# ittiam-systems/libxaac

Hardware: AMD Instinct MI355X
Metric: decoded audio frames/s (1024-spl IMDCT + complex QMF + HQ SBR + parametric stereo, HE-AACv2) (higher is better)
Workload: dtype int32

## Files before the change

### libxaac_amd/csrc/sbr_core_kernel.hip

```cpp
#include <hip/hip_runtime.h>
#include <stddef.h>
#include <stdint.h>
#include <stdlib.h>

#ifdef XS_PROFILE
__shared__ long long xs_prof_last[4];
__shared__ unsigned xs_prof_acc[4][32];
#define XS_T(i)                                                  \
  do {                                                           \
    if ((threadIdx.x & 63) == 0) {                               \
      long long t_ = clock64();                                  \
      xs_prof_acc[threadIdx.x >> 6][i] += (unsigned)(t_ - xs_prof_last[threadIdx.x >> 6]); \
      xs_prof_last[threadIdx.x >> 6] = t_;                       \
    }                                                            \
  } while (0)
#endif
__shared__ int16_t xs_lds_inv_table[256];
__shared__ int16_t xs_lds_sqrt_table[258];
__shared__ int32_t xs_lds_rand_ph[568];
__shared__ int16_t xs_lds_rand_hi[568];
__shared__ int16_t xs_lds_small16[8 + 4 + 50];
__shared__ int32_t xs_lds_new_bw[16];
#define XS_TAB_LIMG(i) xs_lds_small16[i]
#define XS_TAB_SMOOTH(i) xs_lds_small16[8 + (i)]
#define XS_TAB_INVINT(i) xs_lds_small16[12 + (i)]
#define XS_TAB_NEWBW(i) xs_lds_new_bw[i]
#define XS_TAB_RAND(i) xs_lds_rand_ph[i]
#define XS_SYNC_WAVE_LDS 1
#define XS_TAB_INV(i) xs_lds_inv_table[i]
#define XS_TAB_SQRT(i) xs_lds_sqrt_table[i]
#include "sbr_core.h"
#include "sbr_core_kernel.h"

#ifndef XS_STAGGER_G
#define XS_STAGGER_G 64
#endif
#ifndef XS_STAGGER_SLEEP
#define XS_STAGGER_SLEEP 16
#endif

namespace {

__device__ __forceinline__ void xs_wave_sync() {
  __builtin_amdgcn_fence(__ATOMIC_RELEASE, "wavefront");
  __builtin_amdgcn_wave_barrier();
  __builtin_amdgcn_fence(__ATOMIC_ACQUIRE, "wavefront");
}

struct XsLdsState {
  int16_t codec_usb, syn_lsb, syn_usb, pad2_;
  XAAC_SBR_STATE_TAIL_FIELDS
};
constexpr int kHeadOff = offsetof(xaac_sbr_state, codec_usb);
constexpr int kTailOff = offsetof(xaac_sbr_state, lpc_real);
constexpr int kTailWords = (sizeof(xaac_sbr_state) - kTailOff) / 4;
static_assert(kHeadOff % 4 == 0 && kTailOff % 4 == 0 && sizeof(xaac_sbr_state) % 4 == 0, "word copies");
static_assert(offsetof(XsLdsState, lpc_real) == 8 && sizeof(XsLdsState) == 8 + kTailWords * 4, "mirror layout");
static_assert(offsetof(xaac_sbr_state, overlap) % 16 == 0 || true, "");
static_assert(sizeof(xaac_sbr_header) % 4 == 0 && sizeof(xaac_sbr_frame) % 4 == 0, "word copies");

constexpr int kFrameHeadBytes = offsetof(xaac_sbr_frame, int_env_sf_arr);
static_assert(kFrameHeadBytes % 4 == 0 && offsetof(xaac_sbr_frame, int_noise_floor) % 4 == 0, "word copies");
static_assert(offsetof(xaac_sbr_frame, int_noise_floor) == kFrameHeadBytes + sizeof(((xaac_sbr_frame *)0)->int_env_sf_arr),
              "nothing but the two arrays behind the head");

template <int HQ, int NB>
struct XsLds {
  typedef XsQmfT<HQ, NB> Q;
  int32_t x[XAAC_SBR_X_ROWS * Q::ROW + (HQ ? 0 : 128)];
  XsLdsState st;
  xaac_sbr_header h;
  int32_t f_head[kFrameHeadBytes / 4];
  int32_t noise_floor[sizeof(((xaac_sbr_frame *)0)->int_noise_floor) / 4];
  XsWork w;
#ifdef XS_LDS_PAD
  char occupancy_probe[XS_LDS_PAD];
#endif
};

__device__ __forceinline__ void copy_words(int32_t *dst, const int32_t *src, int n, int lane) {
  int i = lane;
  for (; i + 64 * 7 < n; i += 64 * 8) {
    int32_t t[8];
#pragma unroll
    for (int j = 0; j < 8; j++) t[j] = src[i + 64 * j];
#pragma unroll
    for (int j = 0; j < 8; j++) dst[i + 64 * j] = t[j];
  }
  int32_t t[8];
#pragma unroll
  for (int j = 0; j < 8; j++)
    if (i + 64 * j < n) t[j] = src[i + 64 * j];
#pragma unroll
  for (int j = 0; j < 8; j++)
    if (i + 64 * j < n) dst[i + 64 * j] = t[j];
}

template <int HQ, int NB, int NS = 32>
__device__ __forceinline__ bool core_one(const XaacSbrCoreParams &p, const int ch, XsLds<HQ, NB> &s, const int lane) {
  typedef XsQmfT<HQ, NB, 0, NS> Q;
  constexpr int ROW = Q::ROW, ROWG = HQ ? 128 : 64, XWG = (HQ ? 2 : 1) * XAAC_SBR_X_WORDS;
  if (NS != 32 && __builtin_amdgcn_readfirstlane((int)p.syn_par[8 * (size_t)ch + 7])) {
    if (lane == 0) {
      p.syn_par[8 * (size_t)ch + 6] = 1;
      if (p.status) p.status[ch] = -1;
    }
    return true;
  }
  xaac_sbr_state *gst = p.state + ch;
  int32_t *gx = p.x + (size_t)ch * XWG;
  const int32_t *gstw = reinterpret_cast<const int32_t *>(gst);

#ifdef XS_PROFILE
  if (lane == 0) {
    for (int i = 0; i < 32; i++) xs_prof_acc[threadIdx.x >> 6][i] = 0;
    xs_prof_last[threadIdx.x >> 6] = clock64();
  }
#endif
  constexpr int NH = (sizeof(xaac_sbr_header) / 4 + 63) / 64, NF = (kFrameHeadBytes / 4 + 63) / 64;
  constexpr int NT = (kTailWords + 63) / 64, NOV = 6 * ROWG / 64, NAS = NS * 32 * (HQ ? 2 : 1) / 64;
  static_assert(NAS * 64 == NS * 32 * (HQ ? 2 : 1), "whole runs of lanes");
  constexpr int NNF = sizeof(s.noise_floor) / 4;
  static_assert(NOV * 64 == 6 * ROWG && NF == 1, "whole rows of lanes");
  constexpr int NSF = (sizeof(((xaac_sbr_frame *)0)->int_env_sf_arr) / 4 + 63) / 64;
  int32_t r_h[NH], r_f, r_nf = 0, r_hd = 0, r_t[NT], r_ov[NOV], r_an[NAS], r_sf[NSF];
  {
    const int32_t *gh = reinterpret_cast<const int32_t *>(p.header + ch), *gf = reinterpret_cast<const int32_t *>(p.frame + ch);
#pragma unroll
    for (int j = 0; j < NH; j++) r_h[j] = lane + 64 * j < (int)(sizeof(xaac_sbr_header) / 4) ? gh[lane + 64 * j] : 0;
    r_f = lane < kFrameHeadBytes / 4 ? gf[lane] : 0;
    if (lane < NNF) r_nf = reinterpret_cast<const int32_t *>(p.frame[ch].int_noise_floor)[lane];
#pragma unroll
    for (int j = 0; j < NSF; j++)
      r_sf[j] = lane + 64 * j < (int)(sizeof(((xaac_sbr_frame *)0)->int_env_sf_arr) / 4) ? reinterpret_cast<const int32_t *>(p.frame[ch].int_env_sf_arr)[lane + 64 * j] : 0;
    if (lane < 2) r_hd = gstw[kHeadOff / 4 + lane];
#pragma unroll
    for (int j = 0; j < NT; j++) r_t[j] = lane + 64 * j < kTailWords ? gstw[kTailOff / 4 + lane + 64 * j] : 0;
    const int32_t *gov = gstw + offsetof(xaac_sbr_state, overlap) / 4;
#pragma unroll
    for (int j = 0; j < NOV; j++) r_ov[j] = gov[lane + 64 * j];
#pragma unroll
    for (int j = 0; j < NAS; j++) {
      const int i = lane + 64 * j;
      const int row = HQ ? (i >> 6) : (i >> 5), col = HQ ? ((i & 31) + ((i & 32) ? 64 : 0)) : (i & 31);
      r_an[j] = gx[(8 + row) * ROWG + col];
    }
  }
  const xaac_sbr_frame *f = reinterpret_cast<const xaac_sbr_frame *>(s.f_head);
  int32_t above = 0;
  {
#pragma unroll
    for (int j = 0; j < NH; j++)
      if (lane + 64 * j < (int)(sizeof(xaac_sbr_header) / 4)) reinterpret_cast<int32_t *>(&s.h)[lane + 64 * j] = r_h[j];
    if (lane < kFrameHeadBytes / 4) s.f_head[lane] = r_f;
    if (lane < NNF) s.noise_floor[lane] = r_nf;
    int32_t *m = reinterpret_cast<int32_t *>(&s.st);
    if (lane < 2) m[lane] = r_hd;
#pragma unroll
    for (int j = 0; j < NT; j++)
      if (lane + 64 * j < kTailWords) m[2 + lane + 64 * j] = r_t[j];
    for (int i = lane; i < 2 * ROW; i += 64) s.x[i] = 0;
    if (NS < 32)
      for (int i = lane; i < (32 - NS) * ROW; i += 64) s.x[(8 + NS) * ROW + i] = 0;
    if (!HQ)
      for (int i = lane; i < 128; i += 64) s.x[XAAC_SBR_X_ROWS * ROW + i] = 0;
  }
  const bool held = NB == 64 || lane < NB;
#pragma unroll
  for (int j = 0; j < NOV; j++) above |= held ? 0 : r_ov[j];
  auto store_matrix = [&]() {
    if (held) {
#pragma unroll
      for (int j = 0; j < NOV; j++) {
        const int row = HQ ? j >> 1 : j, part = HQ ? j & 1 : 0;
        s.x[(2 + row) * ROW + part * NB + lane] = r_ov[j];
      }
    }
#pragma unroll
    for (int j = 0; j < NAS; j++) {
      const int i = lane + 64 * j;
      const int row = HQ ? (i >> 6) : (i >> 5), col = HQ ? ((i & 31) + ((i & 32) ? Q::IM : 0)) : (i & 31);
      s.x[(8 + row) * ROW + col] = r_an[j];
    }
    for (int i = lane; i < NS * (HQ ? 2 : 1) * (NB - 32); i += 64) {
      const int row = i / ((HQ ? 2 : 1) * (NB - 32)), c = i % ((HQ ? 2 : 1) * (NB - 32));
      s.x[(8 + row) * ROW + (c < NB - 32 ? 32 + c : Q::IM + 32 + (c - (NB - 32)))] = 0;
    }
  };
  xs_wave_sync();
#ifdef XS_PROFILE
  XS_T(24);
#endif

  const XsCx cx = {lane, 64};
  const Q x = {s.x};
  if (lane == 0) s.st.lb_scale = 0;
  const int refused = xs_side_info_bad(cx, &s.h, f, &s.st, 0, NS);
  if (NB < 64) {
    int32_t top = 0;
    if (!refused) {
      const int32_t lim[4] = {s.st.syn_usb, s.st.syn_lsb, s.st.codec_usb, s.st.prev_max_qmf_subband_aac};
      for (int i = 0; i < 4; i++) top = lim[i] > top ? lim[i] : top;
      if (f->apply_processing) {
        top = s.h.sub_band_end > top ? s.h.sub_band_end : top;
        top = f->max_qmf_subband_aac > top ? f->max_qmf_subband_aac : top;
        if (lane <= s.h.num_sf_bands[1] && s.h.freq_band_tbl_hi[lane] > top) top = s.h.freq_band_tbl_hi[lane];
        if (lane <= s.h.num_sf_bands[0] && s.h.freq_band_tbl_lo[lane] > top) top = s.h.freq_band_tbl_lo[lane];
        if (lane < s.h.num_patches) {
          const xaac_sbr_patch *pp = &s.h.patch[lane];
          const int a = pp->src_end_band + pp->dst_end_band, b = pp->dst_start_band + pp->num_bands_in_patch;
          top = a > top ? a : top;
          top = b > top ? b : top;
        }
      }
    }
    if (cx.wave_max(top) > NB || cx.wave_or(above) != 0) return false;
  }
  const int apply = __builtin_amdgcn_readfirstlane((int)f->apply_processing);
  const int old_lsb = __builtin_amdgcn_readfirstlane((int)s.st.prev_max_qmf_subband_aac);
  const int new_lsb = __builtin_amdgcn_readfirstlane((int)f->max_qmf_subband_aac);
  const bool in_regs = !refused && !(apply && new_lsb != old_lsb && old_lsb > 0);
  if (!in_regs) store_matrix();
  if (apply && !refused) xs_rescale_x_overlap(cx, &s.h, f, &s.st, x);
  xs_wave_sync();
  if (lane == 0) {
    s.st.st_lb_scale = 0;
    s.st.lb_scale = HQ ? -8 : -10;
  }
  xs_wave_sync();
  int save_lb_scale = 0;
  XsPendingAdjust pend = {0, 0, 0, 0, 0};
  XS_T(26);
#ifdef XS_SKIP_CORE
  const int rc = 0;
  if (in_regs) store_matrix();
#else
  int rc = -1;
  if (in_regs) {
    const int usb = __builtin_amdgcn_readfirstlane((int)s.st.codec_usb);
    int32_t m_ov = 1, m_an = 1;
    const bool low_ov = lane < usb, low_an = (lane & 31) < usb;
#pragma unroll
    for (int j = 0; j < NOV; j++) m_ov |= low_ov ? fx_abs_nrm(r_ov[j]) : 0;
#pragma unroll
    for (int j = 0; j < NAS; j++) m_an |= low_an ? fx_abs_nrm(r_an[j]) : 0;
    const int reserve = xs_pnorm32(cx.wave_or(m_an)), reserve_ov1 = xs_pnorm32(cx.wave_or(m_ov));
    const XsBfp b = xs_bfp_shifts<HQ>(cx, &s.st, usb, reserve, reserve_ov1);
    if (b.sh_ov != 0) {
#pragma unroll
      for (int j = 0; j < NOV; j++) r_ov[j] = low_ov ? xs_adjust_word(r_ov[j], b.sh_ov) : r_ov[j];
    }
    if (b.sh_main != 0) {
#pragma unroll
      for (int j = 0; j < NAS; j++) r_an[j] = low_an ? xs_adjust_word(r_an[j], b.sh_main) : r_an[j];
    }
    store_matrix();
    save_lb_scale = b.save_lb_scale;
    xs_wave_sync();
    XS_T(1);
    rc = xs_sbr_core_tail(cx, &s.h, f, p.frame[ch].int_env_sf_arr, reinterpret_cast<const int16_t *>(s.noise_floor), &s.st, x,
                          &s.w, HQ ? nullptr : xs_lds_rand_hi, b, &pend, r_sf);
  } else if (!refused) {
    rc = xs_sbr_core(cx, &s.h, f, p.frame[ch].int_env_sf_arr, reinterpret_cast<const int16_t *>(s.noise_floor), &s.st, x, &s.w,
                     HQ ? nullptr : xs_lds_rand_hi, &save_lb_scale);
  }
#endif
  xs_wave_sync();
#ifdef XS_PROFILE
  XS_T(15);
#endif

  if (lane == 0) {
    int16_t *par = p.syn_par + 8 * (size_t)ch;
    par[0] = s.st.lb_scale;
    par[1] = s.st.ov_lb_scale;
    par[2] = s.st.hb_scale;
    par[3] = s.st.st_syn_scale;
    par[4] = s.st.syn_lsb;
    par[5] = s.st.syn_usb;
    par[6] = 0;
    par[7] = 0;
    s.st.ov_lb_scale = (int16_t)save_lb_scale;
#ifndef XS_PROFILE
    if (p.status) p.status[ch] = rc;
#endif
  }
  xs_wave_sync();
  {
    constexpr int NW = (NS + 6) * ROWG / 64;
    const bool held = NB == 64 || lane < NB;
    const int lane_h = held ? lane : 0;
    const bool adj_band = lane >= pend.b0 && lane < pend.b1;
    const auto counts = [](int sh, int &l, int &r) {
      sh = sh > 31 ? 31 : (sh < -31 ? -31 : sh);
      l = sh > 0 ? sh : 0;
      r = sh < 0 ? -sh : 0;
    };
    int ov_l, ov_r, mn_l, mn_r;
    counts(pend.sh_ov, ov_l, ov_r);
    counts(pend.sh_main, mn_l, mn_r);
#pragma unroll
    for (int j0 = 0; j0 < NW; j0 += 8) {
      int32_t t[8];
#pragma unroll
      for (int j = 0; j < 8; j++)
        if (j0 + j < NW) {
          const int row = HQ ? (j0 + j) >> 1 : j0 + j, part = HQ ? (j0 + j) & 1 : 0;
          int32_t v = s.x[(2 + row) * ROW + part * NB + lane_h];
          if (row < NS) {
            const int sl = row < pend.first_start ? ov_l : mn_l, sr = row < pend.first_start ? ov_r : mn_r;
            const int32_t w = (int32_t)((uint32_t)v << sl) >> sr;
            v = adj_band ? w : v;
          }
          t[j] = held ? v : 0;
        }
#pragma unroll
      for (int j = 0; j < 8; j++)
        if (j0 + j < NW) gx[2 * ROWG + 64 * (j0 + j) + lane] = t[j];
    }
  }
  {
    int32_t *gw = reinterpret_cast<int32_t *>(gst);
#pragma unroll
    for (int j = 0; j < 6; j++) {
      const int row = HQ ? j >> 1 : j, part = HQ ? j & 1 : 0;
      const bool held = NB == 64 || lane < NB;
      int32_t v = s.x[(2 + NS + row) * ROW + part * NB + (held ? lane : 0)];
      if (NS + row < pend.first_start && lane >= pend.b0 && lane < pend.b1) {
        const int sh = pend.sh_ov > 31 ? 31 : (pend.sh_ov < -31 ? -31 : pend.sh_ov);
        v = sh > 0 ? (int32_t)((uint32_t)v << sh) : (v >> -sh);
      }
      gw[offsetof(xaac_sbr_state, overlap) / 4 + 64 * j + lane] = held ? v : 0;
    }
    const int32_t *m = reinterpret_cast<const int32_t *>(&s.st);
    if (lane < 2) gw[kHeadOff / 4 + lane] = m[lane];
    copy_words(gw + kTailOff / 4, m + 2, kTailWords, lane);
  }
#ifdef XS_PROFILE
  XS_T(25);
  xs_wave_sync();
  if (lane < 32 && p.status) atomicAdd(reinterpret_cast<unsigned long long *>(p.status) + lane, (unsigned long long)xs_prof_acc[threadIdx.x >> 6][lane]);
#endif
  return true;
}

template <int HQ, int THREADS>
__device__ __forceinline__ void stage_tables(int tid) {
  constexpr int NR = (568 + THREADS - 1) / THREADS, NI = (256 + THREADS - 1) / THREADS, NS = (257 + THREADS - 1) / THREADS;
  int32_t tr[NR];
  int16_t ti[NI], ts[NS];
  const auto upto = [](int i, int n) { return i < n ? i : n - 1; };
#pragma unroll
  for (int j = 0; j < NR; j++) tr[j] = xaac_sbr_rand_ph[upto(tid + THREADS * j, 568)];
#pragma unroll
  for (int j = 0; j < NI; j++) ti[j] = xaac_sbr_inv_table[upto(tid + THREADS * j, 256)];
#pragma unroll
  for (int j = 0; j < NS; j++) ts[j] = xaac_sbr_sqrt_table[upto(tid + THREADS * j, 257)];
  const int16_t s_lim = xaac_sbr_lim_gains_m[upto(tid, 8)], s_smooth = xaac_sbr_smooth_filter[upto(tid - 8 < 0 ? 0 : tid - 8, 4)];
  const int16_t s_inv = xaac_sbr_inv_int_table[upto(tid - 12 < 0 ? 0 : tid - 12, 49)];
  const int32_t s_bw = xaac_sbr_new_bw_table[upto(tid, 16)];
  if (tid < 8) xs_lds_small16[tid] = s_lim;
  if (tid >= 8 && tid < 12) xs_lds_small16[tid] = s_smooth;
  if (tid >= 12 && tid < 12 + 49) xs_lds_small16[tid] = s_inv;
  if (tid < 16) xs_lds_new_bw[tid] = s_bw;
#pragma unroll
  for (int j = 0; j < NR; j++)
    if (tid + THREADS * j < 568) {
      if (HQ)
        xs_lds_rand_ph[tid + THREADS * j] = tr[j];
      else
        xs_lds_rand_hi[tid + THREADS * j] = (int16_t)(tr[j] >> 16);
    }
#pragma unroll
  for (int j = 0; j < NI; j++)
    if (tid + THREADS * j < 256) xs_lds_inv_table[tid + THREADS * j] = ti[j];
#pragma unroll
  for (int j = 0; j < NS; j++)
    if (tid + THREADS * j < 257) xs_lds_sqrt_table[tid + THREADS * j] = ts[j];
}

}

#ifndef XS_LP_MIN_WAVES
#define XS_LP_MIN_WAVES 3
#endif
template <int HQ, int NB, int WAVES, int NS = 32>
__global__ __launch_bounds__(64 * WAVES, HQ ? 1 : XS_LP_MIN_WAVES) void xaac_sbr_core_kernel(XaacSbrCoreParams p) {
  __shared__ XsLds<HQ, NB> s[WAVES];
  const int lane = threadIdx.x & 63, wave = __builtin_amdgcn_readfirstlane(threadIdx.x >> 6);
  stage_tables<HQ, 64 * WAVES>(threadIdx.x);
  __syncthreads();
  if (XS_STAGGER_G > 1 && p.work_counter && p.n_ch >= 3 * (int)gridDim.x * WAVES) {
    const int g = ((int)blockIdx.x * WAVES + wave) % XS_STAGGER_G;
    for (int t = 0; t < g; t++) __builtin_amdgcn_s_sleep(XS_STAGGER_SLEEP);
  }
  for (bool first = true;; first = false) {
    int ch = 0;
    if (p.work_counter) {
      if (lane == 0) ch = atomicAdd(p.work_counter, 1);
      ch = __builtin_amdgcn_readfirstlane(ch);
    } else {
      ch = first ? (int)blockIdx.x * WAVES + wave : p.n_ch;
    }
    if (ch >= p.n_ch) break;
    if (!core_one<HQ, NB, NS>(p, ch, s[wave], lane) && lane == 0) {
      if (p.narrow_only) {
        if (p.status) p.status[ch] = XAAC_FATAL_BAD_ARG;
      } else {
        p.defer_list[atomicAdd(p.defer_count, 1)] = ch;
      }
    }
    xs_wave_sync();
  }
}

template <int HQ, int NS = 32>
__global__ __launch_bounds__(64) void xaac_sbr_core_list_kernel(XaacSbrCoreParams p) {
  __shared__ XsLds<HQ, 64> s;
  const int lane = threadIdx.x;
  const int n = *p.defer_count;
  if ((int)blockIdx.x >= n) return;
  stage_tables<HQ, 64>(lane);
  for (int j = blockIdx.x; j < n; j += gridDim.x) {
    xs_wave_sync();
    core_one<HQ, 64, NS>(p, p.defer_list[j], s, lane);
  }
}

template <int NS>
static hipError_t launch_sbr_core_lp(const XaacSbrCoreParams *p, hipStream_t stream) {
  XaacSbrCoreParams q = *p;
  q.work_counter = nullptr;
#ifndef XS_LP_WAVES
#define XS_LP_WAVES 2
#endif
  constexpr int W = XS_LP_WAVES;
#ifndef XS_LP_PERSISTENT
#define XS_LP_PERSISTENT 1
#endif
  if (XS_LP_PERSISTENT && p->work_counter && p->counters_zeroed) {
#ifndef XS_LP_WG_PER_CU
#define XS_LP_WG_PER_CU 5
#endif
    const int resident = XS_LP_WG_PER_CU * (p->num_cu > 0 ? p->num_cu : 256), need = (p->n_ch + W - 1) / W;
    hipLaunchKernelGGL((xaac_sbr_core_kernel<0, 64, W, NS>), dim3(need < resident ? need : resident), dim3(64 * W), 0, stream, *p);
    return hipGetLastError();
  }
  hipLaunchKernelGGL((xaac_sbr_core_kernel<0, 64, W, NS>), dim3((p->n_ch + W - 1) / W), dim3(64 * W), 0, stream, q);
  return hipGetLastError();
}

template <int NS>
__global__ __launch_bounds__(256) void xaac_sbr_screen_kernel(XaacSbrCoreParams p) {
  const int lane = threadIdx.x & 63, ch = __builtin_amdgcn_readfirstlane((int)(blockIdx.x * 4 + (threadIdx.x >> 6)));
  if (ch >= p.n_ch) return;
  const XsCx cx = {lane, 64};
  const int bad = xs_side_info_bad(cx, p.header + ch, p.frame + ch, p.state + ch, 0, NS);
  if (lane == 0) p.syn_par[8 * (size_t)ch + 7] = (int16_t)(bad ? 1 : 0);
}

extern "C" hipError_t xaac_launch_sbr_screen(const XaacSbrCoreParams *p, hipStream_t stream) {
  if (p->qmf_slots != 30) return hipErrorInvalidValue;
  hipLaunchKernelGGL((xaac_sbr_screen_kernel<30>), dim3((p->n_ch + 3) / 4), dim3(256), 0, stream, *p);
  return hipGetLastError();
}

extern "C" hipError_t xaac_launch_sbr_core_lp(const XaacSbrCoreParams *p, hipStream_t stream) {
  return p->qmf_slots == 30 ? launch_sbr_core_lp<30>(p, stream) : launch_sbr_core_lp<32>(p, stream);
}

template <int NS>
static hipError_t launch_sbr_core_hq(const XaacSbrCoreParams *p, hipStream_t stream) {
  if (!p->defer_list || !p->defer_count || !p->work_counter) {
    XaacSbrCoreParams q = *p;
    q.work_counter = nullptr;
    hipLaunchKernelGGL((xaac_sbr_core_kernel<1, 64, 1, NS>), dim3(p->n_ch), dim3(64), 0, stream, q);
    return hipGetLastError();
  }
  if (!p->counters_zeroed) {
    hipError_t e = hipMemsetAsync(p->defer_count, 0, 2 * sizeof(int32_t), stream);
    if (e != hipSuccess) return e;
  }
  constexpr int W = XAAC_SBR_CORE_HQ_WAVES;
  static int per_cu = 0;
  if (!per_cu) {
    const char *e = getenv("XAAC_CORE_WG_PER_CU");
    per_cu = e && atoi(e) > 0 ? atoi(e) : 2;
  }
  const int resident = per_cu * (p->num_cu > 0 ? p->num_cu : 256), need = (p->n_ch + W - 1) / W;
  hipLaunchKernelGGL((xaac_sbr_core_kernel<1, XAAC_SBR_NARROW_BANDS, W, NS>), dim3(need < resident ? need : resident), dim3(64 * W), 0,
                     stream, *p);
  if (p->narrow_only) return hipGetLastError();
  const int grid = p->n_ch < 64 ? p->n_ch : 64;
  hipLaunchKernelGGL((xaac_sbr_core_list_kernel<1, NS>), dim3(grid), dim3(64), 0, stream, *p);
  return hipGetLastError();
}

extern "C" hipError_t xaac_launch_sbr_core_hq(const XaacSbrCoreParams *p, hipStream_t stream) {
  return p->qmf_slots == 30 ? launch_sbr_core_hq<30>(p, stream) : launch_sbr_core_hq<32>(p, stream);
}

extern "C" hipError_t xaac_warm_sbr_core(void) {
  hipFuncAttributes a;
  return hipFuncGetAttributes(&a, reinterpret_cast<const void *>(&xaac_sbr_core_kernel<1, XAAC_SBR_NARROW_BANDS, XAAC_SBR_CORE_HQ_WAVES, 32>));
}
```

Baseline: 18.30 million.

## Unify SBR core paths and specialize output shift loop by uniform mode

Removes the separate xs_sbr_core fallback, so the non-register path computes headroom and adjusts the matrix in LDS before calling the shared core tail. Headroom is now found from per-lane max/min instead of a per-element abs-norm. Register shifts run as uniform shift loops, and the LDS zero-fill is a strided loop with no division. The output copy is instantiated per wave-uniform shift mode, which drops per-element selects in the common case. It also adds asm phase markers for profiling. The aim is lower ALU cost and smaller code, at the risk of more template instantiations and a behaviour change on the fallback path.

Result: no change. 18.28 million (-0.1%).

```diff
diff --git a/libxaac_amd/csrc/sbr_core_kernel.hip b/libxaac_amd/csrc/sbr_core_kernel.hip
--- a/libxaac_amd/csrc/sbr_core_kernel.hip
+++ b/libxaac_amd/csrc/sbr_core_kernel.hip
@@ -2,6 +2,7 @@
 #include <stddef.h>
 #include <stdint.h>
 #include <stdlib.h>
+#include <type_traits>
 
 #ifdef XS_PROFILE
 __shared__ long long xs_prof_last[4];
@@ -14,6 +15,8 @@
       xs_prof_last[threadIdx.x >> 6] = t_;                       \
     }                                                            \
   } while (0)
+#elif defined(XS_PHASE_MARKS)
+#define XS_T(i) asm volatile("; XS_PHASE " #i)
 #endif
 __shared__ int16_t xs_lds_inv_table[256];
 __shared__ int16_t xs_lds_sqrt_table[258];
@@ -166,8 +169,11 @@
       for (int i = lane; i < 128; i += 64) s.x[XAAC_SBR_X_ROWS * ROW + i] = 0;
   }
   const bool held = NB == 64 || lane < NB;
-#pragma unroll
-  for (int j = 0; j < NOV; j++) above |= held ? 0 : r_ov[j];
+  if (NB < 64) {
+#pragma unroll
+    for (int j = 0; j < NOV; j++) above |= r_ov[j];
+    above = held ? 0 : above;
+  }
   auto store_matrix = [&]() {
     if (held) {
 #pragma unroll
@@ -182,13 +188,22 @@
       const int row = HQ ? (i >> 6) : (i >> 5), col = HQ ? ((i & 31) + ((i & 32) ? Q::IM : 0)) : (i & 31);
       s.x[(8 + row) * ROW + col] = r_an[j];
     }
-    for (int i = lane; i < NS * (HQ ? 2 : 1) * (NB - 32); i += 64) {
-      const int row = i / ((HQ ? 2 : 1) * (NB - 32)), c = i % ((HQ ? 2 : 1) * (NB - 32));
-      s.x[(8 + row) * ROW + (c < NB - 32 ? 32 + c : Q::IM + 32 + (c - (NB - 32)))] = 0;
+    constexpr int ZC = (HQ ? 2 : 1) * (NB - 32);
+    if constexpr (ZC > 0 && 64 % (ZC > 0 ? ZC : 1) == 0 && NS % (64 / (ZC > 0 ? ZC : 1)) == 0) {
+      constexpr int ZR = 64 / ZC;
+      const int c = lane % ZC;
+      int32_t *z = &s.x[(8 + lane / ZC) * ROW + (c < NB - 32 ? 32 + c : Q::IM + 32 + (c - (NB - 32)))];
+#pragma unroll
+      for (int k = 0; k < NS / ZR; k++) z[k * ZR * ROW] = 0;
+    } else {
+      for (int i = lane; i < NS * ZC; i += 64) {
+        const int row = i / (ZC > 0 ? ZC : 1), c = i % (ZC > 0 ? ZC : 1);
+        s.x[(8 + row) * ROW + (c < NB - 32 ? 32 + c : Q::IM + 32 + (c - (NB - 32)))] = 0;
+      }
     }
   };
   xs_wave_sync();
-#ifdef XS_PROFILE
+#if defined(XS_PROFILE) || defined(XS_PHASE_MARKS)
   XS_T(24);
 #endif
 
@@ -236,37 +251,55 @@
   if (in_regs) store_matrix();
 #else
   int rc = -1;
-  if (in_regs) {
+  if (!refused) {
     const int usb = __builtin_amdgcn_readfirstlane((int)s.st.codec_usb);
-    int32_t m_ov = 1, m_an = 1;
-    const bool low_ov = lane < usb, low_an = (lane & 31) < usb;
-#pragma unroll
-    for (int j = 0; j < NOV; j++) m_ov |= low_ov ? fx_abs_nrm(r_ov[j]) : 0;
-#pragma unroll
-    for (int j = 0; j < NAS; j++) m_an |= low_an ? fx_abs_nrm(r_an[j]) : 0;
-    const int reserve = xs_pnorm32(cx.wave_or(m_an)), reserve_ov1 = xs_pnorm32(cx.wave_or(m_ov));
-    const XsBfp b = xs_bfp_shifts<HQ>(cx, &s.st, usb, reserve, reserve_ov1);
-    if (b.sh_ov != 0) {
-#pragma unroll
-      for (int j = 0; j < NOV; j++) r_ov[j] = low_ov ? xs_adjust_word(r_ov[j], b.sh_ov) : r_ov[j];
-    }
-    if (b.sh_main != 0) {
-#pragma unroll
-      for (int j = 0; j < NAS; j++) r_an[j] = low_an ? xs_adjust_word(r_an[j], b.sh_main) : r_an[j];
-    }
-    store_matrix();
+    XsBfp b;
+    if (in_regs) {
+      int32_t hi_ov = 0, lo_ov = -1, hi_an = 0, lo_an = -1;
+      const bool low_ov = lane < usb, low_an = (lane & 31) < usb;
+#pragma unroll
+      for (int j = 0; j < NOV; j++) {
+        hi_ov = r_ov[j] > hi_ov ? r_ov[j] : hi_ov;
+        lo_ov = r_ov[j] < lo_ov ? r_ov[j] : lo_ov;
+      }
+#pragma unroll
+      for (int j = 0; j < NAS; j++) {
+        hi_an = r_an[j] > hi_an ? r_an[j] : hi_an;
+        lo_an = r_an[j] < lo_an ? r_an[j] : lo_an;
+      }
+      const int32_t m_ov = (low_ov ? hi_ov | ~lo_ov : 0) | 1, m_an = (low_an ? hi_an | ~lo_an : 0) | 1;
+      const int reserve = xs_pnorm32(cx.wave_or(m_an)), reserve_ov1 = xs_pnorm32(cx.wave_or(m_ov));
+      b = xs_bfp_shifts<HQ>(cx, &s.st, usb, reserve, reserve_ov1);
+      const auto adjust = [](int32_t *r, const int n, const bool low, int sh) {
+        sh = sh > 31 ? 31 : (sh < -31 ? -31 : sh);
+        if (sh > 0) {
+          const int l = low ? sh : 0;
+#pragma unroll
+          for (int j = 0; j < n; j++) r[j] = fx_shlw(r[j], l);
+        } else if (sh < 0) {
+          const int l = low ? -sh : 0;
+#pragma unroll
+          for (int j = 0; j < n; j++) r[j] >>= l;
+        }
+      };
+      adjust(r_ov, NOV, low_ov, b.sh_ov);
+      adjust(r_an, NAS, low_an, b.sh_main);
+      store_matrix();
+    } else {
+      const int reserve = xs_headroom(cx, x, 0, usb, Q::OV, Q::OV + NS), reserve_ov1 = xs_headroom(cx, x, 0, usb, 0, Q::OV);
+      b = xs_bfp_shifts<HQ>(cx, &s.st, usb, reserve, reserve_ov1);
+      xs_adjust(cx, x, 0, usb, 0, Q::OV, b.sh_ov);
+      xs_adjust(cx, x, 0, usb, Q::OV, Q::OV + NS, b.sh_main);
+    }
     save_lb_scale = b.save_lb_scale;
     xs_wave_sync();
     XS_T(1);
     rc = xs_sbr_core_tail(cx, &s.h, f, p.frame[ch].int_env_sf_arr, reinterpret_cast<const int16_t *>(s.noise_floor), &s.st, x,
                           &s.w, HQ ? nullptr : xs_lds_rand_hi, b, &pend, r_sf);
-  } else if (!refused) {
-    rc = xs_sbr_core(cx, &s.h, f, p.frame[ch].int_env_sf_arr, reinterpret_cast<const int16_t *>(s.noise_floor), &s.st, x, &s.w,
-                     HQ ? nullptr : xs_lds_rand_hi, &save_lb_scale);
   }
 #endif
   xs_wave_sync();
-#ifdef XS_PROFILE
+#if defined(XS_PROFILE) || defined(XS_PHASE_MARKS)
   XS_T(15);
 #endif
 
@@ -299,25 +332,42 @@
     int ov_l, ov_r, mn_l, mn_r;
     counts(pend.sh_ov, ov_l, ov_r);
     counts(pend.sh_main, mn_l, mn_r);
-#pragma unroll
-    for (int j0 = 0; j0 < NW; j0 += 8) {
-      int32_t t[8];
-#pragma unroll
-      for (int j = 0; j < 8; j++)
-        if (j0 + j < NW) {
-          const int row = HQ ? (j0 + j) >> 1 : j0 + j, part = HQ ? (j0 + j) & 1 : 0;
-          int32_t v = s.x[(2 + row) * ROW + part * NB + lane_h];
-          if (row < NS) {
-            const int sl = row < pend.first_start ? ov_l : mn_l, sr = row < pend.first_start ? ov_r : mn_r;
-            const int32_t w = (int32_t)((uint32_t)v << sl) >> sr;
-            v = adj_band ? w : v;
+    const auto rows_out = [&](auto mode) {
+      constexpr int MODE = decltype(mode)::value;
+      const int cnt = MODE == 1 ? (adj_band ? mn_r : 0) : (adj_band ? mn_l : 0);
+#pragma unroll
+      for (int j0 = 0; j0 < NW; j0 += 8) {
+        int32_t t[8];
+#pragma unroll
+        for (int j = 0; j < 8; j++)
+          if (j0 + j < NW) {
+            const int row = HQ ? (j0 + j) >> 1 : j0 + j, part = HQ ? (j0 + j) & 1 : 0;
+            int32_t v = s.x[(2 + row) * ROW + part * NB + lane_h];
+            if (row < NS) {
+              if (MODE == 1) v >>= cnt;
+              if (MODE == 2) v = (int32_t)((uint32_t)v << cnt);
+              if (MODE == 3) {
+                const int sl = row < pend.first_start ? ov_l : mn_l, sr = row < pend.first_start ? ov_r : mn_r;
+                const int32_t w = (int32_t)((uint32_t)v << sl) >> sr;
+                v = adj_band ? w : v;
+              }
+            }
+            t[j] = held ? v : 0;
           }
-          t[j] = held ? v : 0;
-        }
-#pragma unroll
-      for (int j = 0; j < 8; j++)
-        if (j0 + j < NW) gx[2 * ROWG + 64 * (j0 + j) + lane] = t[j];
-    }
+#pragma unroll
+        for (int j = 0; j < 8; j++)
+          if (j0 + j < NW) gx[2 * ROWG + 64 * (j0 + j) + lane] = t[j];
+      }
+    };
+    const int mode = __builtin_amdgcn_readfirstlane(pend.first_start > 0 ? 3 : (mn_r != 0 ? 1 : (mn_l != 0 ? 2 : 0)));
+    if (mode == 3)
+      rows_out(std::integral_constant<int, 3>());
+    else if (mode == 1)
+      rows_out(std::integral_constant<int, 1>());
+    else if (mode == 2)
+      rows_out(std::integral_constant<int, 2>());
+    else
+      rows_out(std::integral_constant<int, 0>());
   }
   {
     int32_t *gw = reinterpret_cast<int32_t *>(gst);
@@ -336,8 +386,10 @@
     if (lane < 2) gw[kHeadOff / 4 + lane] = m[lane];
     copy_words(gw + kTailOff / 4, m + 2, kTailWords, lane);
   }
+#if defined(XS_PROFILE) || defined(XS_PHASE_MARKS)
+  XS_T(25);
+#endif
 #ifdef XS_PROFILE
-  XS_T(25);
   xs_wave_sync();
   if (lane < 32 && p.status) atomicAdd(reinterpret_cast<unsigned long long *>(p.status) + lane, (unsigned long long)xs_prof_acc[threadIdx.x >> 6][lane]);
 #endif
```
